# MarbleHE/ABC

Measured on AMD Instinct MI355X. Metric: homomorphic mul+relin/sec, CKKS N=2^14, higher is better.
Workload: dtype u64 (transforms: exact integer arithmetic in f64); 1 GPU; CKKS N=16384, 4 data limbs {50,40,40,40} + special 50-bit prime, ct x ct multiply + relinearize; total_batch=8192, batch_rank0=8192

## Files before the change

abc_amd/csrc/abc_context.hip:

```cpp
#include <cstdlib>
#include <cstring>
#include <mutex>

#include "../../include/abc_hip.h"
#include <dlfcn.h>

#include "abc_context.hpp"
#include "abc_host_math.hpp"
#include "abc_sample.hpp"

namespace abc {

static thread_local std::string g_err;
void set_error(const std::string &msg) { g_err = msg; }

static bool env_on(const char *name) {
  const char *e = std::getenv(name);
  return e && !(e[0] == '0' && e[1] == 0);
}
void read_switches(abc_hip_ctx *c) {
  abc_hip_ctx::Switches s;
  s.no_fused = env_on("ABC_HIP_NO_FUSED");
  s.no_split = env_on("ABC_HIP_NO_SPLIT");
  s.no_split4 = env_on("ABC_HIP_NO_SPLIT4");
  s.no_isplit = env_on("ABC_HIP_NO_ISPLIT");
  s.no_gsplit = env_on("ABC_HIP_NO_GSPLIT");
  s.no_bsplit = env_on("ABC_HIP_NO_BSPLIT");
  s.no_mixed = env_on("ABC_HIP_NO_MIXED");
  s.no_pack = env_on("ABC_HIP_NO_PACK");
  s.no_key_twin = env_on("ABC_HIP_NO_KEY_TWIN");
  s.no_bmul = env_on("ABC_HIP_NO_BMUL");
  s.no_iks = env_on("ABC_HIP_NO_IKS");
  s.no_lean_front = env_on("ABC_HIP_NO_LEAN_FRONT");
  s.no_tensor_intt = env_on("ABC_HIP_NO_TENSOR_INTT");
  s.no_galois_fusion = env_on("ABC_HIP_NO_GALOIS_FUSION");
  s.host_sampling = env_on("ABC_HIP_HOST_SAMPLING");
  if (const char *e = std::getenv("ABC_HIP_CHUNK")) s.chunk = (size_t)std::atol(e);
  if (const char *e = std::getenv("ABC_HIP_FEW_LIMBS")) s.few_limbs = (size_t)std::atol(e);
  if (const char *e = std::getenv("ABC_HIP_LEAN_LIMIT")) s.lean_limit = (size_t)std::atol(e);
  if (const char *e = std::getenv("ABC_HIP_PASS0_TARGET_LIMIT")) s.pass0_target_limit = (size_t)std::atol(e);
  if (const char *e = std::getenv("ABC_HIP_BFV_SCRATCH_MB")) s.bfv_scratch_mb = (size_t)std::atol(e);
  if (const char *e = std::getenv("ABC_HIP_LANES")) {
    s.lanes = std::atoi(e);
    if (s.lanes < 1) s.lanes = 1;
    if (s.lanes > abc_hip_ctx::kMaxLanes) s.lanes = abc_hip_ctx::kMaxLanes;
  }
  c->sw = s;
  RouteFacts &f = c->facts;
  f = RouteFacts{};
  f.scheme = c->scheme; f.logn = c->logn; f.K = c->K; f.L = c->L; f.nB = c->nB;
  f.use_fp = c->use_fp; f.behz_fp = c->behz_fp;
  f.big_block_log = big_block_log();
  for (int j = 0; j < c->K; j++) f.bits[j] = (unsigned char)c->h_mods[j].bits;
  f.sw = s;
  f.finish();
}

static Mod make_mod(uint64_t q, int logn, bool ntt) {
  using namespace host;
  Mod m{};
  m.q = q;
  m.two_q = 2 * q;
  const int k = bitlen(q);
  m.bits = (u32)k;
  m.shift = (u32)(k - 1);
  m.mu = (uint64_t)((((u128)1) << (k + 63)) / q);
  m.qd = (double)q;
  m.qinv = 1.0 / (double)q;
  if (ntt) {
    const uint64_t n = 1ull << logn;
    m.inv_n = invmod(n % q, q);
    m.inv_n_s = shoup(m.inv_n, q);
    if (fp_ok(m.bits)) {
      m.inv_n_c = m.inv_n > q / 2 ? -(double)(q - m.inv_n) : (double)m.inv_n;
      m.inv_n_cq = m.inv_n_c / m.qd;
    }
  }
  return m;
}

static void fill_twiddles(uint64_t q, int logn, uint64_t *dst ) {
  using namespace host;
  const size_t n = (size_t)1 << logn;
  const uint64_t psi = min_primitive_root(2 * n, q);
  uint64_t *fwd = dst, *inv = dst + 2 * n;
  uint64_t p = 1;
  for (size_t i = 0; i < n; i++) {
    fwd[2 * (size_t)bitrev((uint32_t)i, logn)] = p;
    p = mulmod(p, psi, q);
  }
  const uint64_t ipsi = invmod(psi, q);
  p = 1;
  for (size_t i = 0; i < n; i++) {
    inv[2 * (size_t)bitrev((uint32_t)i, logn)] = p;
    p = mulmod(p, ipsi, q);
  }
  for (size_t i = 0; i < n; i++) {
    fwd[2 * i + 1] = shoup(fwd[2 * i], q);
    inv[2 * i + 1] = shoup(inv[2 * i], q);
  }
}

static void fill_fp_twiddles(uint64_t q, size_t n, const uint64_t *src , double *dst ) {
  for (size_t i = 0; i < 2 * n; i++) {
    const uint64_t w = src[2 * i];
    dst[i] = w > q / 2 ? -(double)(q - w) : (double)w;
  }
}

static int build_context(abc_hip_ctx *c) {
  using namespace host;
  const int logn = c->logn, K = c->K, L = c->L;
  const size_t N = (size_t)c->n;
  const bool bfv = (c->scheme == ABC_HIP_SCHEME_BFV);
  std::vector<uint64_t> qs(c->primes.begin(), c->primes.begin() + L);
  const uint64_t qsp = c->primes[K - 1];
  DevConst &k = c->h_cst;
  std::memset(&k, 0, sizeof(k));

  c->mod_values.assign(c->primes.begin(), c->primes.end());
  std::vector<uint64_t> Bp;
  uint64_t m_sk = 0, gamma = 0;
  if (bfv) {
    bool fp_aux = !env_on("ABC_HIP_NO_FP64") && !env_on("ABC_HIP_BEHZ_SEAL_BASE");
    for (uint64_t q : c->primes) fp_aux = fp_aux && fp_ok((u32)bitlen(q));
    const int aux_bits = fp_aux ? 50 : 61;
    int nB = L;
    if (32 + bitlen(c->t) + prod_bitlen(qs) >= aux_bits * L + aux_bits) nB++;
    gamma = ntt_primes(N, 61, 2)[1];
    if (!fp_aux) {
      auto aux = ntt_primes(N, 61, (size_t)nB + 2);
      m_sk = aux[0];
      Bp.assign(aux.begin() + 2, aux.end());
    } else {
      std::vector<uint64_t> alt;
      for (uint64_t p : ntt_primes(N, 50, (size_t)nB + 1 + (size_t)K)) {
        bool clash = false;
        for (uint64_t q : c->primes) clash = clash || (p == q);
        if (!clash && alt.size() < (size_t)nB + 1) alt.push_back(p);
      }
      if (alt.size() < (size_t)nB + 1) throw std::runtime_error("not enough 50-bit NTT primes for the BEHZ auxiliary base");
      m_sk = alt[0];
      Bp.assign(alt.begin() + 1, alt.end());
    }
    c->behz_fp = fp_aux && L <= 10 && !env_on("ABC_HIP_BEHZ_INT_KERNELS");
    c->nB = nB;
    c->nBsk = nB + 1;
    for (uint64_t b : Bp) c->mod_values.push_back(b);
    c->mod_values.push_back(m_sk);
    c->mod_values.push_back(gamma);
    c->mod_values.push_back(c->t);
  }
  const int nmods = (int)c->mod_values.size();
  const int id_bsk = K, id_gamma = K + c->nBsk, id_t = K + c->nBsk + 1;
  c->h_mods.clear();
  std::vector<uint64_t> h_tw((size_t)nmods * 4 * N, 0);
  std::vector<double> h_ftw((size_t)nmods * 2 * N, 0.0);
  for (int i = 0; i < nmods; i++) {
    const bool ntt = !(bfv && i == id_gamma);
    c->h_mods.push_back(make_mod(c->mod_values[i], logn, ntt));
    if (ntt) fill_twiddles(c->mod_values[i], logn, h_tw.data() + (size_t)i * 4 * N);
    if (ntt && fp_ok(c->h_mods.back().bits))
      fill_fp_twiddles(c->mod_values[i], N, h_tw.data() + (size_t)i * 4 * N, h_ftw.data() + (size_t)i * 2 * N);
  }

  for (int j = 0; j < L; j++) {
    const uint64_t q = qs[j];
    k.inv_special[j] = invmod(qsp % q, q);
    k.inv_special_s[j] = shoup(k.inv_special[j], q);
    k.special_mod_q[j] = qsp % q;
    k.special_mod_q_s[j] = shoup(k.special_mod_q[j], q);
    k.inv_special_c[j] = k.inv_special[j] > q / 2 ? -(double)(q - k.inv_special[j]) : (double)k.inv_special[j];
    k.inv_special_cq[j] = k.inv_special_c[j] / (double)q;
    k.special_c[j] = k.special_mod_q[j] > q / 2 ? -(double)(q - k.special_mod_q[j]) : (double)k.special_mod_q[j];
    k.special_cq[j] = k.special_c[j] / (double)q;
  }
  for (int l = 1; l < L; l++)
    for (int j = 0; j < l; j++) {
      k.inv_qlast[l][j] = invmod(qs[l] % qs[j], qs[j]);
      k.inv_qlast_s[l][j] = shoup(k.inv_qlast[l][j], qs[j]);
      k.inv_qlast_c[l][j] = k.inv_qlast[l][j] > qs[j] / 2 ? -(double)(qs[j] - k.inv_qlast[l][j]) : (double)k.inv_qlast[l][j];
      k.inv_qlast_cq[l][j] = k.inv_qlast_c[l][j] / (double)qs[j];
    }

  std::vector<uint32_t> slot_map;
  if (bfv) {
    const uint64_t t = c->t;
    k.t = t;
// ... 767 lines not shown
```

abc_amd/csrc/abc_kernels_fused.hip:

```cpp
#include <type_traits>

#include "abc_context.hpp"
#include "abc_host_math.hpp"

namespace abc {

template <int LB>
__global__ __launch_bounds__((1 << LB) / 16) void k_fused_tensor_intt(DevCtx c, const u64 *__restrict__ a,
                                                                      const u64 *__restrict__ b, u64 *__restrict__ c01,
                                                                      u64 *__restrict__ c2coef, u64 *__restrict__ c2ntt, int nl) {
  __shared__ u64 lds[lds_words(LB)];
  const int j = blockIdx.x % nl;
  const size_t ct = blockIdx.x / nl;
  const size_t N = (size_t)1 << LB, pw = (size_t)nl * N;
  const Mod m = c.mods[j];
  const NttTable t = ntt_table(c, j);
  const u64 *__restrict__ a0 = a + ct * 2 * pw + j * N, *__restrict__ a1 = a0 + pw;
  const u64 *__restrict__ b0 = b + ct * 2 * pw + j * N, *__restrict__ b1 = b0 + pw;
  u64 *__restrict__ o0 = c01 + ct * 2 * pw + j * N, *__restrict__ o1 = o0 + pw;
  u64 *__restrict__ dcoef = c2coef + (ct * nl + j) * N, *__restrict__ dntt = c2ntt + (ct * nl + j) * N;
  ntt_inv_block<LB>(
      lds,
      [&](int, int i) {
        const u64 x0 = a0[i], x1 = a1[i], y0 = b0[i], y1 = b1[i];
// ... 602 lines not shown
  const size_t cc = blockIdx.x >> 2;
  const int p = (int)((blockIdx.x & 3) << 8) + (int)threadIdx.x;
  const int hi0[1] = {0};
  double x[16];
  {
    const Mod ms = mod_at(c, c.K - 1);
    const FpTable ts = fp_table(c, c.K - 1);
    const FpK ks = FpArith::consts(ms);
    const double *__restrict__ src = tsp_half + cc * (size_t)c.ps;
#pragma unroll
    for (int k = 0; k < 16; k++) x[k] = src[(k << 10) + p];
    FpArith::centre16(x, ks);
    inv_pass<FpArith, LB, 0, 4>(x, hi0, ts, ks, 0, 0);
    const double half = (double)(ms.q >> 1);
#pragma unroll
    for (int k = 0; k < 16; k++) {
      const double w = fp_centre(fp_mul_lazy(x[k], ms.inv_n_c, ms.inv_n_cq, ms.qd) + half, ms.qd, ms.qinv);
      x[k] = w < 0.0 ? w + ms.qd : w;
    }
  }
  const u64 half = c.mods[c.K - 1].q >> 1;
  for (int j = 0; j < nl; j++) {
    const Mod m = mod_at(c, j);
    const FpTable t = fp_table(c, j);
    const FpK kk = FpArith::consts(m);
    const u64 hm = reduce64(half, m);
    const double fix = hm ? (double)(m.q - hm) : 0.0;
    double y[16];
#pragma unroll
    for (int k = 0; k < 16; k++) y[k] = x[k] + fix;
    fwd_pass<FpArith, LB, 0, 4>(y, hi0, t, kk, 0, 0);
    double *__restrict__ dst = tpart + (cc * nl + j) * (size_t)c.ps;
    store_half_done<LB>(dst, y, p, kk, pack ? pack_kind(m.bits) : 0);
  }
}

template <int MODE, bool GAL, int NL>
__global__ __launch_bounds__(NL ? (NL + 1) * 64 : 832) void k_split3_main_fp(DevCtx c, const double *__restrict__ part,
                                                                              const double *__restrict__ tpart,
                                                                              const u64 *__restrict__ opa, const u64 *__restrict__ opb,
                                                                              size_t opa_stride, size_t opb_stride, int add_c1,
                                                                              const u64 *__restrict__ key, u64 *__restrict__ out, int nl_rt,
                                                                              u32 gelt) {
  extern __shared__ double dyn[];
  const int nl = NL ? NL : nl_rt;
  const int W = __builtin_amdgcn_readfirstlane((int)(threadIdx.x >> 6));
  const int lane = threadIdx.x & 63;
  const int blk = blockIdx.x & 15;
  const int I = (int)((blockIdx.x >> 4) % nl);
  const size_t ct = (size_t)((blockIdx.x >> 4) / nl);
  const size_t N = (size_t)c.n, base = (size_t)blk << 10;
  const Mod m = mod_at(c, I);
  const FpTable t = fp_table(c, I);
  const double q = m.qd, qinv = m.qinv;
  {
    double *buf = dyn + W * lds_words(10);
    const double *__restrict__ src;
    if (W < nl - 1) {
      const int J = W < I ? W : W + 1;
      src = part + ((ct * (nl + 1) + I) * nl + J) * (size_t)c.ps + base;
    } else {
      src = tpart + ((ct * 2 + (W - (nl - 1))) * nl + I) * (size_t)c.ps + base;
    }
    ntt_fwd_block_a<10, FpArith>(
        buf, [&](int, int i) { return fp_centre(src[i], q, qinv); }, [&](int, int i, double v) { buf[lds_pad(i)] = v; }, t, m, 4, blk,
        lane);
  }
  __syncthreads();
  const double inv = c.cst->inv_special_c[I], inv_q = c.cst->inv_special_cq[I];
  const size_t pw = (size_t)nl * N;
  const double *tt0 = dyn + (nl - 1) * lds_words(10), *tt1 = dyn + nl * lds_words(10);
  for (int e = 2 * (int)threadIdx.x; e < 1024; e += 2 * (int)blockDim.x) {
    double s0[2] = {0.0, 0.0}, s1[2] = {0.0, 0.0}, d0[2] = {0.0, 0.0}, d1[2] = {0.0, 0.0};
#pragma unroll
    for (int Jx = 0; Jx < (NL ? NL : 12); Jx++) {
      if (!NL && Jx >= nl) break;
      double x[2];
      if (Jx == I) {
        if (MODE == 0) {
          const u64 *pa = opa + ct * 2 * pw + (size_t)I * N + base + e, *pb = opb + ct * 2 * pw + (size_t)I * N + base + e;
          const u64x2 a0 = *reinterpret_cast<const u64x2 *>(pa), a1 = *reinterpret_cast<const u64x2 *>(pa + pw);
          const u64x2 b0 = *reinterpret_cast<const u64x2 *>(pb), b1 = *reinterpret_cast<const u64x2 *>(pb + pw);
          const double x0[2] = {fp_from_u64(a0.x), fp_from_u64(a0.y)}, x1[2] = {fp_from_u64(a1.x), fp_from_u64(a1.y)};
          const double y0[2] = {fp_from_u64(b0.x), fp_from_u64(b0.y)}, y1[2] = {fp_from_u64(b1.x), fp_from_u64(b1.y)};
#pragma unroll
          for (int k = 0; k < 2; k++) {
            x[k] = fp_mulmod(x1[k], y1[k], q, qinv);
            d0[k] = fp_mulmod(x0[k], y0[k], q, qinv);
            d1[k] = fp_mulmod(x0[k], y1[k], q, qinv) + fp_mulmod(x1[k], y0[k], q, qinv);
          }
        } else {
          const u64 *xl = opa + ct * opa_stride + (size_t)I * N;
#pragma unroll
          for (int k = 0; k < 2; k++) {
            const u32 si = galois_ntt_src<GAL>((u32)(base + e + k), gelt, c.logn);
            x[k] = fp_from_u64(xl[si]);
            if (opb) {
              const u64 *ad = opb + ct * opb_stride + (size_t)I * N;
              d0[k] = fp_from_u64(ad[si]);
              if (add_c1) d1[k] = fp_from_u64(ad[pw + si]);
            }
          }
        }
      } else {
        const int w = Jx < I ? Jx : Jx - 1;
        const f64x2 v = *reinterpret_cast<const f64x2 *>(dyn + w * lds_words(10) + lds_pad(e));
        x[0] = v.x;
        x[1] = v.y;
      }
      const u64x2 k0 = *reinterpret_cast<const u64x2 *>(key + (((size_t)Jx * 2 + 0) * c.K + I) * N + base + e);
      const u64x2 k1 = *reinterpret_cast<const u64x2 *>(key + (((size_t)Jx * 2 + 1) * c.K + I) * N + base + e);
      s0[0] += fp_mulmod(x[0], fp_from_u64(k0.x), q, qinv);
      s0[1] += fp_mulmod(x[1], fp_from_u64(k0.y), q, qinv);
      s1[0] += fp_mulmod(x[0], fp_from_u64(k1.x), q, qinv);
      s1[1] += fp_mulmod(x[1], fp_from_u64(k1.y), q, qinv);
      if (Jx == 7) {
#pragma unroll
        for (int k = 0; k < 2; k++) {
          s0[k] = fp_centre(s0[k], q, qinv);
          s1[k] = fp_centre(s1[k], q, qinv);
        }
      }
    }
    const f64x2 u0 = *reinterpret_cast<const f64x2 *>(tt0 + lds_pad(e)), u1 = *reinterpret_cast<const f64x2 *>(tt1 + lds_pad(e));
    u64x2 r;
    r.x = fp_to_canon(fp_mul_lazy(s0[0] - u0.x, inv, inv_q, q) + d0[0], q, qinv);
    r.y = fp_to_canon(fp_mul_lazy(s0[1] - u0.y, inv, inv_q, q) + d0[1], q, qinv);
    *reinterpret_cast<u64x2 *>(out + ((ct * 2 + 0) * nl + I) * N + base + e) = r;
    r.x = fp_to_canon(fp_mul_lazy(s1[0] - u1.x, inv, inv_q, q) + d1[0], q, qinv);
    r.y = fp_to_canon(fp_mul_lazy(s1[1] - u1.y, inv, inv_q, q) + d1[1], q, qinv);
    *reinterpret_cast<u64x2 *>(out + ((ct * 2 + 1) * nl + I) * N + base + e) = r;
  }
}

template <int MODE, bool GAL>
static void launch_split3_main(abc_hip_ctx *c, const MainArgs &a) {
  const int nl = a.nl;
  const dim3 grid((unsigned)(a.cc * nl * 16)), block(64 * (nl + 1));
  const size_t lds = (size_t)((nl + 1) * lds_words(10)) * 8;
#define ABC_TM3(NLV)                                                                                                             \
  hipLaunchKernelGGL((k_split3_main_fp<MODE, GAL, NLV>), grid, block, lds, a.st, c->dc, (const double *)a.part, (const double *)a.tpart, \
                     a.opa, a.opb, a.opa_stride, a.opb_stride, a.add_c1, a.key, a.out, nl, a.gelt)
  switch (nl) {
    case 1: ABC_TM3(1); break;
    case 2: ABC_TM3(2); break;
    case 3: ABC_TM3(3); break;
    case 4: ABC_TM3(4); break;
    default: ABC_TM3(0); break;
  }
#undef ABC_TM3
}


template <int MODE, int NL>
struct PairOps {
  u64x2 k0[NL], k1[NL];
  u64x2 a0, a1, b0, b1;
  u64 xs[2], d0s[2], d1s[2];
};

template <int MODE, bool GAL, int NL>
__global__ __launch_bounds__(512, NL <= 4 ? 4 : 2) void k_split4_main_fp(DevCtx c, const double *__restrict__ part,
                                                                   const double *__restrict__ tpart, const u64 *__restrict__ opa,
                                                                   const u64 *__restrict__ opb, size_t opa_stride, size_t opb_stride,
                                                                   int add_c1, const u64 *__restrict__ key, u64 *__restrict__ out, u32 gelt,
                                                                   u32 imap, int ni, int pack, const double *__restrict__ keyf) {
  extern __shared__ double dyn[];
  static_assert(NL + 1 <= 8, "one wavefront per limb, eight wavefronts");
  constexpr int nl = NL, NT = 512, PER = 2;
  constexpr int LATE = (MODE == 0 && NL == 4) ? 1 : 0;
  const int W = __builtin_amdgcn_readfirstlane((int)(threadIdx.x >> 6));
  const int lane = threadIdx.x & 63;
  const int blk = blockIdx.x & 15;
  const int I = (int)((imap >> (4 * ((blockIdx.x >> 4) % (unsigned)ni))) & 15u);
  const size_t ct = (size_t)((blockIdx.x >> 4) / (unsigned)ni);
  const size_t N = (size_t)c.n, base = (size_t)blk << 10;
  const Mod m = mod_at(c, I);
  const FpTable t = fp_table(c, I);
  const double q = m.qd, qinv = m.qinv;
  double *ltw = dyn + (nl + 1) * lds_words(10);
  const size_t pw = (size_t)nl * N;
  const ABC_CONST_AS DevConst *cst = (const ABC_CONST_AS DevConst *)c.cst;
  const double inv = cst->inv_special_c[I], inv_q = cst->inv_special_cq[I];

  double twv[PER];
  block_twiddles_fetch<10, double, PER>(t.tw, 4, blk, (int)threadIdx.x, NT, twv);
  const bool has_limb = W <= nl;
  const int Wc = has_limb ? W : 0;
  const double *__restrict__ src = (Wc < nl - 1) ? part + ((ct * (nl + 1) + I) * nl + (Wc < I ? Wc : Wc + 1)) * (size_t)c.ps + base
                                                 : tpart + ((ct * 2 + (Wc - (nl - 1))) * nl + I) * (size_t)c.ps + base;
  const int pk = pack ? pack_kind(m.bits) : 0;
  u64x2 raw[8];
  if (has_limb) {
    if (pk == 0) {
#pragma unroll
      for (int k = 0; k < 8; k++) raw[k] = *reinterpret_cast<const u64x2 *>(src + (k << 7) + 2 * lane);
    } else if (pk == 1) {
#pragma unroll
      for (int k = 0; k < 8; k++) raw[k] = pack_load_pair<1>(src - base, N, base + (k << 7) + 2 * lane);
    } else {
#pragma unroll
      for (int k = 0; k < 8; k++) raw[k] = pack_load_pair<2>(src - base, N, base + (k << 7) + 2 * lane);
    }
  }
  auto load_key = [&](int e, PairOps<MODE, NL> &o, int j0, int j1) {
    const u64 *kw = keyf ? reinterpret_cast<const u64 *>(keyf) : key;
#pragma unroll
    for (int Jx = 0; Jx < NL; Jx++) {
      if (Jx < j0 || Jx >= j1) continue;
      o.k0[Jx] = *reinterpret_cast<const u64x2 *>(kw + (((size_t)Jx * 2 + 0) * c.K + I) * N + base + e);
      o.k1[Jx] = *reinterpret_cast<const u64x2 *>(kw + (((size_t)Jx * 2 + 1) * c.K + I) * N + base + e);
    }
  };
  auto load_pair = [&](int e, PairOps<MODE, NL> &o) {
    load_key(e, o, 0, NL - LATE);
    if (MODE == 0) {
      const u64 *pa = opa + ct * 2 * pw + (size_t)I * N + base + e, *pb = opb + ct * 2 * pw + (size_t)I * N + base + e;
      o.a0 = *reinterpret_cast<const u64x2 *>(pa); o.a1 = *reinterpret_cast<const u64x2 *>(pa + pw);
      o.b0 = *reinterpret_cast<const u64x2 *>(pb); o.b1 = *reinterpret_cast<const u64x2 *>(pb + pw);
    } else {
      const u64 *xl = opa + ct * opa_stride + (size_t)I * N;
#pragma unroll
      for (int k = 0; k < 2; k++) {
        const u32 si = galois_ntt_src<GAL>((u32)(base + e + k), gelt, c.logn);
        o.xs[k] = xl[si];
        o.d0s[k] = o.d1s[k] = 0;
        if (opb) {
          const u64 *ad = opb + ct * opb_stride + (size_t)I * N;
          o.d0s[k] = ad[si];
          if (add_c1) o.d1s[k] = ad[pw + si];
        }
      }
    }
  };
  PairOps<MODE, NL> ops;
  load_pair(2 * (int)threadIdx.x, ops);

  block_twiddles_store<10, double, PER>(ltw, (int)threadIdx.x, NT, twv);
  __syncthreads();
  if (has_limb) {
    double *buf = dyn + W * lds_words(10);
    double xin[16];
    if (pk == 0) {
#pragma unroll
      for (int k = 0; k < 8; k++) {
        xin[k] = __longlong_as_double((long long)raw[k].x);
        xin[8 + k] = __longlong_as_double((long long)raw[k].y);
      }
    } else if (pk == 1) {
#pragma unroll
      for (int k = 0; k < 8; k++) pack_decode_pair<1>(raw[k], xin[k], xin[8 + k]);
    } else {
#pragma unroll
      for (int k = 0; k < 8; k++) pack_decode_pair<2>(raw[k], xin[k], xin[8 + k]);
    }
    if (m.bits >= 49) {
#pragma unroll
      for (int r = 0; r < 16; r++) xin[r] = fp_centre(xin[r], q, qinv);
    }
    ntt_fwd_tail1024_pairs<FpTail>(buf, xin, [&](int, int i, double v) { buf[lds_pad(i)] = v; }, t, m, 4, blk, lane, ltw);
  }
  if (LATE) load_key(2 * (int)threadIdx.x, ops, NL - LATE, NL);
  __syncthreads();
  const double *tt0 = dyn + (nl - 1) * lds_words(10), *tt1 = dyn + nl * lds_words(10);
  auto compute_pair = [&](int e, const PairOps<MODE, NL> &o, auto twin) {
    constexpr bool TW = decltype(twin)::value;
    auto kd = [](u64 w) { return TW ? __longlong_as_double((long long)w) : fp_from_u64(w); };
    double s0[2] = {0.0, 0.0}, s1[2] = {0.0, 0.0}, d0[2] = {0.0, 0.0}, d1[2] = {0.0, 0.0};
#pragma unroll
    for (int Jx = 0; Jx < NL; Jx++) {
      double x[2];
      if (Jx == I) {
        if (MODE == 0) {
          const double x0[2] = {fp_from_u64(o.a0.x), fp_from_u64(o.a0.y)}, x1[2] = {fp_from_u64(o.a1.x), fp_from_u64(o.a1.y)};
          const double y0[2] = {fp_from_u64(o.b0.x), fp_from_u64(o.b0.y)}, y1[2] = {fp_from_u64(o.b1.x), fp_from_u64(o.b1.y)};
#pragma unroll
          for (int k = 0; k < 2; k++) {
            x[k] = fp_mulmod(x1[k], y1[k], q, qinv);
            d0[k] = fp_mulmod(x0[k], y0[k], q, qinv);
            d1[k] = fp_mulmod(x0[k], y1[k], q, qinv) + fp_mulmod(x1[k], y0[k], q, qinv);
          }
        } else {
#pragma unroll
          for (int k = 0; k < 2; k++) {
            x[k] = fp_from_u64(o.xs[k]);
            d0[k] = fp_from_u64(o.d0s[k]);
            d1[k] = fp_from_u64(o.d1s[k]);
          }
        }
      } else {
        const int w = Jx < I ? Jx : Jx - 1;
        const f64x2 v = *reinterpret_cast<const f64x2 *>(dyn + w * lds_words(10) + lds_pad(e));
        x[0] = v.x;
        x[1] = v.y;
      }
      s0[0] += fp_mulmod(x[0], kd(o.k0[Jx].x), q, qinv);
      s0[1] += fp_mulmod(x[1], kd(o.k0[Jx].y), q, qinv);
      s1[0] += fp_mulmod(x[0], kd(o.k1[Jx].x), q, qinv);
      s1[1] += fp_mulmod(x[1], kd(o.k1[Jx].y), q, qinv);
      if (Jx == 7) {
#pragma unroll
        for (int k = 0; k < 2; k++) {
          s0[k] = fp_centre(s0[k], q, qinv);
          s1[k] = fp_centre(s1[k], q, qinv);
        }
      }
    }
    const f64x2 u0 = *reinterpret_cast<const f64x2 *>(tt0 + lds_pad(e)), u1 = *reinterpret_cast<const f64x2 *>(tt1 + lds_pad(e));
    u64x2 r;
    r.x = fp_to_canon(fp_mul_lazy(s0[0] - u0.x, inv, inv_q, q) + d0[0], q, qinv);
    r.y = fp_to_canon(fp_mul_lazy(s0[1] - u0.y, inv, inv_q, q) + d0[1], q, qinv);
    *reinterpret_cast<u64x2 *>(out + ((ct * 2 + 0) * nl + I) * N + base + e) = r;
    r.x = fp_to_canon(fp_mul_lazy(s1[0] - u1.x, inv, inv_q, q) + d1[0], q, qinv);
    r.y = fp_to_canon(fp_mul_lazy(s1[1] - u1.y, inv, inv_q, q) + d1[1], q, qinv);
    *reinterpret_cast<u64x2 *>(out + ((ct * 2 + 1) * nl + I) * N + base + e) = r;
  };
  if (keyf) compute_pair(2 * (int)threadIdx.x, ops, std::true_type{});
  else compute_pair(2 * (int)threadIdx.x, ops, std::false_type{});
}

bool split4_main(abc_hip_ctx *c, int mode, const MainArgs &a) {
  if (a.nl < 1 || a.nl > 7) return false;
  if (a.ni == 0) return true;
  const dim3 grid((unsigned)(a.cc * a.ni * 16)), block(512);
  const double *keyf = key_twin_lookup(c, a.key);
  dispatch_mode(mode, a.gelt, [&](auto M, auto G) {
    dispatch_nl<1, 7>(a.nl, [&](auto NL) {
      hipLaunchKernelGGL((k_split4_main_fp<decltype(M)::value, decltype(G)::value, decltype(NL)::value>), grid, block, main_lds_bytes(a.nl, sizeof(double)),
                         a.st, c->dc, (const double *)a.part, (const double *)a.tpart, a.opa, a.opb, a.opa_stride, a.opb_stride, a.add_c1,
                         a.key, a.out, a.gelt, (u32)a.imap, a.ni, a.pack, keyf);
    });
  });
  return true;
}

static void launch_split3(abc_hip_ctx *c, const FusedScratch &s, int mode, MainArgs a, bool main4) {
  a.part = s.dec;
  a.tpart = s.ksacc;
  launch_split_special(a.st, c, a.cc, a.nl, (const double *)s.dec, a.key, (double *)s.tsp);
  hipLaunchKernelGGL(k_split3_pass_fp<14>, dim3((unsigned)(a.cc * 2 * 4)), dim3(256), 0, a.st, c->dc, (const double *)s.tsp,
                     (double *)s.ksacc, a.nl, a.pack);
  if (main4 && split4_main(c, mode, a)) return;
  dispatch_mode(mode, a.gelt, [&](auto M, auto G) { launch_split3_main<decltype(M)::value, decltype(G)::value>(c, a); });
}

template <int LB>
static int keyswitch_stage(abc_hip_ctx *c, hipStream_t st, const FusedScratch &s, const u64 *coef, size_t coef_stride, const u64 *ntt,
                           size_t ntt_stride, const u64 *key, const u64 *addend, size_t addend_stride, bool add_c1, u64 *out, int nl,
                           size_t cc, bool fp , const ChunkRoute &k,
                           int dec_ready = 0 ) {
  const size_t N = (size_t)1 << LB;
  const dim3 block((1 << LB) / 16);
  const bool ckks = (c->scheme == 2);
  const bool guard = k.guard, lazy = k.lazy;
  const unsigned g2a = (unsigned)(cc * (nl + 1) * nl);
  const unsigned g3 = (unsigned)(cc * 2 * nl);
  if (fp) {
    if (!dec_ready)
      hipLaunchKernelGGL(k_fused_ks_decomp_ntt_fp<LB>, dim3(g2a), block, 0, st, c->dc, coef, coef_stride, s.dec, nl, ckks ? 1 : 0);
    hipLaunchKernelGGL(k_fused_ks_mac, dim3(grid_for(cc * (nl + 1) * (N / 2), 256)), dim3(256), 0, st, c->dc, s.dec,
                       ckks ? ntt : (const u64 *)nullptr, ntt_stride, key, s.ksacc, s.tsp, nl, cc);
    hipLaunchKernelGGL(k_fused_ks_special_intt_fp<LB>, dim3((unsigned)(cc * 2)), block, 0, st, c->dc, s.tsp, s.tlast);
    if (ckks)
      hipLaunchKernelGGL((k_fused_ks_moddown_fp<LB, false>), dim3(g3), block, 0, st, c->dc, s.ksacc, s.tlast, addend, addend_stride,
                         add_c1 ? 1 : 0, out, nl, (int)(cc * 2), 0u);
    else
      hipLaunchKernelGGL(k_fused_ks_moddown_bfv_fp<LB>, dim3(g3), block, 0, st, c->dc, s.ksacc, s.tlast, addend, addend_stride,
                         add_c1 ? 1 : 0, out, nl);
    ABC_HIP_CHECK(hipGetLastError());
    return 0;
  }
  if (guard)
    hipLaunchKernelGGL((k_fused_ks_decomp_ntt<LB, true, false>), dim3(g2a), block, 0, st, c->dc, coef, coef_stride, s.dec, nl,
                       ckks ? 1 : 0);
  else if (lazy)
    hipLaunchKernelGGL((k_fused_ks_decomp_ntt<LB, false, true>), dim3(g2a), block, 0, st, c->dc, coef, coef_stride, s.dec, nl,
                       ckks ? 1 : 0);
  else
    hipLaunchKernelGGL((k_fused_ks_decomp_ntt<LB, false, false>), dim3(g2a), block, 0, st, c->dc, coef, coef_stride, s.dec, nl,
                       ckks ? 1 : 0);
  hipLaunchKernelGGL(k_fused_ks_mac, dim3(grid_for(cc * (nl + 1) * (N / 2), 256)), dim3(256), 0, st, c->dc, s.dec,
                     ckks ? ntt : (const u64 *)nullptr, ntt_stride, key, s.ksacc, s.tsp, nl, cc);
  hipLaunchKernelGGL(k_fused_ks_special_intt<LB>, dim3((unsigned)(cc * 2)), block, 0, st, c->dc, s.tsp, s.tlast);
  if (!ckks)
    hipLaunchKernelGGL(k_fused_ks_moddown_bfv<LB>, dim3(g3), block, 0, st, c->dc, s.ksacc, s.tlast, addend, addend_stride,
                       add_c1 ? 1 : 0, out, nl);
  else if (guard)
    hipLaunchKernelGGL((k_fused_ks_moddown<LB, true>), dim3(g3), block, 0, st, c->dc, s.ksacc, s.tlast, addend, addend_stride,
                       add_c1 ? 1 : 0, out, nl);
  else
    hipLaunchKernelGGL((k_fused_ks_moddown<LB, false>), dim3(g3), block, 0, st, c->dc, s.ksacc, s.tlast, addend, addend_stride,
                       add_c1 ? 1 : 0, out, nl);
  ABC_HIP_CHECK(hipGetLastError());
  return 0;
}

int fork_lanes(abc_hip_ctx *c, int lanes) {
  if (lanes < 2) return 0;
  ABC_HIP_CHECK(hipEventRecord(c->lane_fork, c->stream));
  for (int l = 0; l < lanes; l++) ABC_HIP_CHECK(hipStreamWaitEvent(c->lane[l], c->lane_fork, 0));
  return 0;
}
int join_lanes(abc_hip_ctx *c, int lanes) {
  if (lanes < 2) return 0;
  for (int l = 0; l < lanes; l++) {
    ABC_HIP_CHECK(hipEventRecord(c->lane_join[l], c->lane[l]));
    ABC_HIP_CHECK(hipStreamWaitEvent(c->stream, c->lane_join[l], 0));
  }
  return 0;
}

static int run_isplit(abc_hip_ctx *c, int mode, const u64 *opa, const u64 *opb, size_t opa_stride, size_t opb_stride, bool add_c1,
                      const u64 *key, u64 *out, int nl, size_t count, u32 gelt) {
  const size_t N = (size_t)c->n;
  const ChunkPlan p = plan_chunks(c->facts, nl, count);
  const ChunkRoute k = route_chunk(c->facts, Seq::isplit, nl, p.chunk);
  return for_each_chunk(c, count, p.chunk, p.lanes, isplit_scratch_words(c, nl), k.fp_twin ? key : nullptr,
                        [&](hipStream_t st, u64 *scratch, size_t off, size_t cc) {
                          return isplit_chunk(c, st, scratch, cc, nl, mode, opa + off * opa_stride, opb ? opb + off * opb_stride : nullptr,
                                              opa_stride, opb_stride, add_c1 ? 1 : 0, key, out + off * 2 * (size_t)nl * N, gelt, k);
                        });
}

static int run_gsplit15(abc_hip_ctx *c, int mode, const u64 *opa, const u64 *opb, size_t opa_stride, size_t opb_stride, bool add_c1,
                        const u64 *key, u64 *out, int nl, size_t count, u32 gelt) {
  const size_t N = (size_t)c->n;
  const ChunkPlan p = plan_chunks(c->facts, nl, count);
  return for_each_chunk(c, count, p.chunk, p.lanes, gsplit_scratch_words(c, nl), nullptr,
                        [&](hipStream_t st, u64 *scratch, size_t off, size_t cc) {
                          return gsplit_chunk15(c, st, scratch, cc, nl, mode, opa + off * opa_stride, opb ? opb + off * opb_stride : nullptr,
                                                opa_stride, opb_stride, add_c1 ? 1 : 0, key, out + off * 2 * (size_t)nl * N, gelt);
                        });
}

template <int LB>
static int run_mul_relin(abc_hip_ctx *c, Seq seq, const u64 *a, const u64 *b, u64 *out, int nl, size_t count) {
  const size_t N = (size_t)1 << LB;
  const ChunkPlan p = plan_chunks(c->facts, nl, count);
  const bool split = seq == Seq::split14, fp = seq != Seq::lds_int;
  const size_t SN = split ? (size_t)c->dc.ps : N;
  const size_t per_ct = fused_scratch_limbs(nl) * SN;
  const size_t ctw = 2 * (size_t)nl * N;
  return for_each_chunk(c, count, p.chunk, p.lanes, per_ct, split ? c->d_relin : nullptr, [&](hipStream_t st, u64 *scratch, size_t off, size_t cc) {
    const FusedScratch s = carve(scratch, p.chunk, nl, SN);
    const ChunkRoute k = route_chunk(c->facts, seq, nl, cc);
    if constexpr (LB == 14) {
      if (split) {
        if (k.lean)
          gsplit_front14(st, c, cc, nl, 0, a + off * ctw, b + off * ctw, 0, (double *)s.coef, (double *)s.dec, 0u, k.pack);
        else
          hipLaunchKernelGGL(k_split2_tensor_pass0_fp<LB>, dim3((unsigned)(cc * nl)), dim3((1 << LB) / 16), 0, st, c->dc, a + off * ctw,
                             b + off * ctw, (double *)s.dec, nl, (int)k.pack);
        launch_split3(c, s, 0, MainArgs{st, cc, nl, nullptr, nullptr, a + off * ctw, b + off * ctw, 0, 0, 0, c->d_relin, out + off * ctw, 0u,
                                        kAllSlots, nl, k.pack},
                      k.main4);
        ABC_HIP_CHECK(hipGetLastError());
        return 0;
      }
    }
    if (fp)
      hipLaunchKernelGGL(k_fused_tensor_decomp_fp<LB>, dim3((unsigned)(cc * nl)), dim3((1 << LB) / 16), 0, st, c->dc, a + off * ctw,
                         b + off * ctw, s.c01, s.ntt, s.dec, nl);
    else
      hipLaunchKernelGGL(k_fused_tensor_intt<LB>, dim3((unsigned)(cc * nl)), dim3((1 << LB) / 16), 0, st, c->dc, a + off * ctw,
                         b + off * ctw, s.c01, s.coef, s.ntt, nl);
    return keyswitch_stage<LB>(c, st, s, s.coef, (size_t)nl * N, s.ntt, (size_t)nl * N, c->d_relin, s.c01, ctw, true, out + off * ctw, nl,
                               cc, fp, k, fp ? 1 : 0);
  });
}

int launch_mul_relin(abc_hip_ctx *c, Seq seq, const u64 *a, const u64 *b, u64 *out, int nl, size_t count) {
  if (!count) return 0;
  const size_t ctw = 2 * (size_t)nl * c->n;
  switch (seq) {
    case Seq::gsplit15: return run_gsplit15(c, 0, a, b, ctw, ctw, false, c->d_relin, out, nl, count, 0u);
    case Seq::isplit: return run_isplit(c, 0, a, b, ctw, ctw, false, c->d_relin, out, nl, count, 0u);
    case Seq::split14:
    case Seq::lds_fp:
    case Seq::lds_int: return dispatch_logn<10, 14>(c->logn, [&](auto LB) { return run_mul_relin<decltype(LB)::value>(c, seq, a, b, out, nl, count); });
    default: set_error("launch_mul_relin: not a multiply + relinearise sequence of this file"); return 1;
  }
}

// ... 79 lines not shown
```

abc_amd/csrc/abc_route.hpp:

```cpp
#pragma once

#include <cstddef>
#include <cstdint>
#include <cstdio>

namespace abc {

struct Switches {
  bool no_fused = false, no_split = false, no_split4 = false, no_isplit = false, no_gsplit = false, no_lean_front = false, no_bsplit = false, no_mixed = false, no_pack = false, no_key_twin = false, no_bmul = false, no_iks = false, no_tensor_intt = false;
  bool no_galois_fusion = false;
  bool host_sampling = false;
  size_t chunk = 0, few_limbs = 48, lean_limit = 96, bfv_scratch_mb = 0, pass0_target_limit = 128;
  int lanes = 2;
};

constexpr unsigned kFpBits = 50;
constexpr unsigned kLazyBits = 55;
constexpr unsigned kUnguardedBits = 57;
constexpr unsigned kIsplitBits = 60;

constexpr size_t fused_scratch_limbs(int nl) { return (size_t)nl * (nl + 1) + 6 * (size_t)nl + 4; }

struct RouteFacts {
  int scheme = 0, logn = 0, K = 0, L = 0, nB = 0;
  bool use_fp = true, behz_fp = false;
  int big_block_log = 12;
  unsigned char bits[17] = {};
  Switches sw;
  unsigned widest = 0;
  uint32_t fp_mask = 0;
  bool all_fp = false;
  bool guard = false;
  bool lazy = false;
  void finish() {
    widest = 0;
    fp_mask = 0;
    for (int j = 0; j < K; j++) {
      if (bits[j] > widest) widest = bits[j];
      if (bits[j] <= kFpBits) fp_mask |= 1u << j;
    }
    all_fp = use_fp && widest <= kFpBits;
    guard = widest > kUnguardedBits;
    lazy = widest <= kLazyBits;
  }
  uint32_t fp_data_mask(int nl) const { return fp_mask & ((1u << nl) - 1u); }
  bool data_fp(int nl) const { return fp_data_mask(nl) == (1u << nl) - 1u; }
  bool special_fp() const { return K > 0 && ((fp_mask >> (K - 1)) & 1u); }
};

enum class Seq {
  split14,
  gsplit15,
  isplit,
  bsplit14,
  bsplit_big,
  lds_fp,
  lds_int,
  bmul,
  generic
};
enum class KsFront { plain, fp, iks };
enum class BfvMul { behz, split, big };
enum class Rescale { generic, fp, mixed };

struct KsRoute {
  Seq seq;
  KsFront front;
};
struct MulRoute {
  Seq seq;
  BfvMul mul;
  KsRoute ks;
};
struct RotRoute {
  bool fold;
  KsRoute ks;
};
struct RescaleRoute {
  Rescale kind;
  uint32_t fpmask;
};

namespace route_detail {
inline bool gsplit_ok(const RouteFacts &f, int nl) {
  return f.logn == 15 && f.scheme == 2 && f.use_fp && !f.sw.no_gsplit && nl >= 1 && nl <= 15 && f.widest <= kFpBits;
}
inline bool bsplit_ok(const RouteFacts &f, int nl) {
  return f.logn == 14 && f.scheme == 1 && f.use_fp && !f.sw.no_bsplit && nl >= 1 && nl <= 8 && f.widest <= kFpBits;
}
inline bool bsplit_big_ok(const RouteFacts &f, int nl) {
  return (f.logn == 13 || f.logn == 15 || f.logn == 16) && f.scheme == 1 && f.use_fp && !f.sw.no_bsplit && !f.sw.no_gsplit && nl >= 1 &&
         nl <= 8 && f.widest <= kFpBits;
}
inline bool isplit_ok(const RouteFacts &f, int nl) {
  if ((f.logn != 14 && f.logn != 15) || f.scheme != 2 || f.sw.no_fused || f.sw.no_split || f.sw.no_isplit || nl < 1 ||
      nl > (f.logn == 15 ? 15 : 7))
    return false;
  if (f.logn == 15 && f.sw.no_gsplit) return false;
  return f.widest <= kIsplitBits;
}
inline bool bmul_shape(const RouteFacts &f, int limbs) {
  return f.scheme == 1 && f.use_fp && f.behz_fp && !f.sw.no_bmul && !f.sw.no_split && !f.sw.no_fused && f.L == limbs && f.nB == limbs &&
         f.K == f.L + 1;
}
inline bool bmul_relin_ok(const RouteFacts &f) {
  if (f.logn == 13) return bmul_shape(f, 4) && bsplit_big_ok(f, f.L);
  return f.logn == 14 && bmul_shape(f, 8) && bsplit_ok(f, f.L);
}
inline Seq lds_seq(const RouteFacts &f, int nl, bool mul) {
  const bool ckks = f.scheme == 2;
  if (f.logn == 14 && ckks && !f.all_fp && isplit_ok(f, nl)) return Seq::isplit;
  if (f.logn == 14 && ckks && f.all_fp && !f.sw.no_split && nl <= 12) return Seq::split14;
  if (!mul && f.logn == 14 && !ckks && !f.sw.no_split && bsplit_ok(f, nl)) return Seq::bsplit14;
  return f.all_fp ? Seq::lds_fp : Seq::lds_int;
}
}

inline KsFront route_ks_front(const RouteFacts &f, int nl) {
  if (f.logn > 14 && f.use_fp && f.data_fp(nl) && f.special_fp()) return KsFront::fp;
  if ((f.logn == 15 || f.logn == 16) && !f.sw.no_iks && f.big_block_log == 12) return KsFront::iks;
  return KsFront::plain;
}

inline KsRoute route_keyswitch(const RouteFacts &f, int nl) {
  using namespace route_detail;
  const KsRoute generic{Seq::generic, route_ks_front(f, nl)};
  if (f.logn == 15 && gsplit_ok(f, nl)) return {Seq::gsplit15, KsFront::plain};
  if (f.logn == 15 && f.scheme == 2 && !f.all_fp && isplit_ok(f, nl)) return {Seq::isplit, KsFront::plain};
  if (bsplit_big_ok(f, nl)) return {Seq::bsplit_big, KsFront::plain};
  if (f.logn > 14 || f.logn < 10 || f.sw.no_fused) return generic;
  return {lds_seq(f, nl, false), KsFront::plain};
}

inline BfvMul route_bfv_multiply(const RouteFacts &f) {
  using namespace route_detail;
  if (f.logn == 14) return bmul_relin_ok(f) ? BfvMul::split : BfvMul::behz;
  if (f.logn == 13) return bmul_shape(f, 4) ? BfvMul::big : BfvMul::behz;
  return ((f.logn == 15 || f.logn == 16) && bmul_shape(f, 8) && !f.sw.no_gsplit && f.big_block_log == 12) ? BfvMul::big : BfvMul::behz;
}

inline MulRoute route_mul_relin(const RouteFacts &f, int nl) {
  using namespace route_detail;
  const KsRoute none{Seq::generic, KsFront::plain};
  if (f.scheme == 2) {
    if (f.logn == 15 && gsplit_ok(f, nl)) return {Seq::gsplit15, BfvMul::behz, none};
    if (f.logn == 15 && !f.all_fp && isplit_ok(f, nl)) return {Seq::isplit, BfvMul::behz, none};
    if (f.logn <= 14 && f.logn >= 10 && !f.sw.no_fused) return {lds_seq(f, nl, true), BfvMul::behz, none};
    return {Seq::generic, BfvMul::behz, route_keyswitch(f, nl)};
  }
  if (bmul_relin_ok(f)) return {Seq::bmul, BfvMul::split, none};
  return {Seq::generic, route_bfv_multiply(f), route_keyswitch(f, nl)};
}

inline RotRoute route_rotate(const RouteFacts &f, int nl, bool in_place) {
  using namespace route_detail;
  const bool may_fold = !in_place && !f.sw.no_galois_fusion;
  if (may_fold && f.logn == 15 && gsplit_ok(f, nl)) return {true, {Seq::gsplit15, KsFront::plain}};
  if (may_fold && f.logn == 15 && f.scheme == 2 && !f.all_fp && isplit_ok(f, nl)) return {true, {Seq::isplit, KsFront::plain}};
  if (may_fold && f.scheme == 1) {
    if (!f.sw.no_split && !f.sw.no_fused) {
      if (f.logn == 14 && bsplit_ok(f, nl)) return {true, {Seq::bsplit14, KsFront::plain}};
      if (bsplit_big_ok(f, nl)) return {true, {Seq::bsplit_big, KsFront::plain}};
    }
// ... 114 lines not shown
```

Measured before the change: 419,000 mul+relin/s.

## Split key-switch main kernel into two output halves for three workgroups per CU

For four or fewer limbs, the split4 main kernel now holds only one key component at a time in registers. It computes the first output component, then reloads the second key component and computes the second. Key and operand loads are also deferred until after the forward NTT, and launch bounds are raised so more workgroups fit per CU. In exchange it adds a second pass over the LDS digits, puts key loads on the critical path, and lets the old schedule be restored with an environment switch.

Measured after the change: 436,000 mul+relin/s, median of 6. 4.1% higher.

```diff
diff --git a/abc_amd/csrc/abc_context.hip b/abc_amd/csrc/abc_context.hip
--- a/abc_amd/csrc/abc_context.hip
+++ b/abc_amd/csrc/abc_context.hip
@@ -34,6 +34,7 @@
   s.no_lean_front = env_on("ABC_HIP_NO_LEAN_FRONT");
   s.no_tensor_intt = env_on("ABC_HIP_NO_TENSOR_INTT");
   s.no_galois_fusion = env_on("ABC_HIP_NO_GALOIS_FUSION");
+  s.main_two_per_cu = env_on("ABC_HIP_MAIN_TWO_PER_CU");
   s.host_sampling = env_on("ABC_HIP_HOST_SAMPLING");
   if (const char *e = std::getenv("ABC_HIP_CHUNK")) s.chunk = (size_t)std::atol(e);
   if (const char *e = std::getenv("ABC_HIP_FEW_LIMBS")) s.few_limbs = (size_t)std::atol(e);
diff --git a/abc_amd/csrc/abc_kernels_fused.hip b/abc_amd/csrc/abc_kernels_fused.hip
--- a/abc_amd/csrc/abc_kernels_fused.hip
+++ b/abc_amd/csrc/abc_kernels_fused.hip
@@ -778,23 +778,25 @@
 }
 
 
-template <int MODE, int NL>
+template <int MODE, int NL, bool HALVES>
 struct PairOps {
-  u64x2 k0[NL], k1[NL];
+  u64x2 k[HALVES ? NL : 2 * NL];
   u64x2 a0, a1, b0, b1;
   u64 xs[2], d0s[2], d1s[2];
 };
 
-template <int MODE, bool GAL, int NL>
-__global__ __launch_bounds__(512, NL <= 4 ? 4 : 2) void k_split4_main_fp(DevCtx c, const double *__restrict__ part,
+template <int MODE, bool GAL, int NL, bool HALVES>
+__global__ __launch_bounds__(512, HALVES ? 6 : NL <= 4 ? 4 : 2) void k_split4_main_fp(DevCtx c, const double *__restrict__ part,
                                                                    const double *__restrict__ tpart, const u64 *__restrict__ opa,
                                                                    const u64 *__restrict__ opb, size_t opa_stride, size_t opb_stride,
                                                                    int add_c1, const u64 *__restrict__ key, u64 *__restrict__ out, u32 gelt,
                                                                    u32 imap, int ni, int pack, const double *__restrict__ keyf) {
   extern __shared__ double dyn[];
   static_assert(NL + 1 <= 8, "one wavefront per limb, eight wavefronts");
+  static_assert(!HALVES || NL <= 4, "three workgroups per CU: four transform buffers at the most");
   constexpr int nl = NL, NT = 512, PER = 2;
-  constexpr int LATE = (MODE == 0 && NL == 4) ? 1 : 0;
+  constexpr int LATE = (!HALVES && MODE == 0 && NL == 4) ? 1 : 0;
+  using Ops = PairOps<MODE, NL, HALVES>;
   const int W = __builtin_amdgcn_readfirstlane((int)(threadIdx.x >> 6));
   const int lane = threadIdx.x & 63;
   const int blk = blockIdx.x & 15;
@@ -829,17 +831,20 @@
       for (int k = 0; k < 8; k++) raw[k] = pack_load_pair<2>(src - base, N, base + (k << 7) + 2 * lane);
     }
   }
-  auto load_key = [&](int e, PairOps<MODE, NL> &o, int j0, int j1) {
+  auto load_key = [&](int e, Ops &o, int j0, int j1, int comp) {
     const u64 *kw = keyf ? reinterpret_cast<const u64 *>(keyf) : key;
 #pragma unroll
     for (int Jx = 0; Jx < NL; Jx++) {
       if (Jx < j0 || Jx >= j1) continue;
-      o.k0[Jx] = *reinterpret_cast<const u64x2 *>(kw + (((size_t)Jx * 2 + 0) * c.K + I) * N + base + e);
-      o.k1[Jx] = *reinterpret_cast<const u64x2 *>(kw + (((size_t)Jx * 2 + 1) * c.K + I) * N + base + e);
+      if constexpr (HALVES) {
+        o.k[Jx] = *reinterpret_cast<const u64x2 *>(kw + (((size_t)Jx * 2 + comp) * c.K + I) * N + base + e);
+      } else {
+        o.k[2 * Jx + 0] = *reinterpret_cast<const u64x2 *>(kw + (((size_t)Jx * 2 + 0) * c.K + I) * N + base + e);
+        o.k[2 * Jx + 1] = *reinterpret_cast<const u64x2 *>(kw + (((size_t)Jx * 2 + 1) * c.K + I) * N + base + e);
+      }
     }
   };
-  auto load_pair = [&](int e, PairOps<MODE, NL> &o) {
-    load_key(e, o, 0, NL - LATE);
+  auto load_operands = [&](int e, Ops &o) {
     if (MODE == 0) {
       const u64 *pa = opa + ct * 2 * pw + (size_t)I * N + base + e, *pb = opb + ct * 2 * pw + (size_t)I * N + base + e;
       o.a0 = *reinterpret_cast<const u64x2 *>(pa); o.a1 = *reinterpret_cast<const u64x2 *>(pa + pw);
@@ -859,8 +864,12 @@
       }
     }
   };
-  PairOps<MODE, NL> ops;
-  load_pair(2 * (int)threadIdx.x, ops);
+  Ops ops;
+  const int e0 = 2 * (int)threadIdx.x;
+  if (!HALVES) {
+    load_key(e0, ops, 0, NL - LATE, 0);
+    load_operands(e0, ops);
+  }
 
   block_twiddles_store<10, double, PER>(ltw, (int)threadIdx.x, NT, twv);
   __syncthreads();
@@ -886,63 +895,97 @@
     }
     ntt_fwd_tail1024_pairs<FpTail>(buf, xin, [&](int, int i, double v) { buf[lds_pad(i)] = v; }, t, m, 4, blk, lane, ltw);
   }
-  if (LATE) load_key(2 * (int)threadIdx.x, ops, NL - LATE, NL);
+  if (HALVES) {
+    load_key(e0, ops, 0, NL, 0);
+    load_operands(e0, ops);
+  }
+  if (LATE) load_key(e0, ops, NL - LATE, NL, 0);
   __syncthreads();
-  const double *tt0 = dyn + (nl - 1) * lds_words(10), *tt1 = dyn + nl * lds_words(10);
-  auto compute_pair = [&](int e, const PairOps<MODE, NL> &o, auto twin) {
+  auto compute_pair = [&](int e, Ops &o, auto twin) {
     constexpr bool TW = decltype(twin)::value;
     auto kd = [](u64 w) { return TW ? __longlong_as_double((long long)w) : fp_from_u64(w); };
-    double s0[2] = {0.0, 0.0}, s1[2] = {0.0, 0.0}, d0[2] = {0.0, 0.0}, d1[2] = {0.0, 0.0};
-#pragma unroll
-    for (int Jx = 0; Jx < NL; Jx++) {
-      double x[2];
-      if (Jx == I) {
-        if (MODE == 0) {
-          const double x0[2] = {fp_from_u64(o.a0.x), fp_from_u64(o.a0.y)}, x1[2] = {fp_from_u64(o.a1.x), fp_from_u64(o.a1.y)};
-          const double y0[2] = {fp_from_u64(o.b0.x), fp_from_u64(o.b0.y)}, y1[2] = {fp_from_u64(o.b1.x), fp_from_u64(o.b1.y)};
+    double xd[2], d0[2] = {0.0, 0.0}, d1[2] = {0.0, 0.0};
+    auto diagonal = [&]() {
+      if (MODE == 0) {
+        const double x0[2] = {fp_from_u64(o.a0.x), fp_from_u64(o.a0.y)}, x1[2] = {fp_from_u64(o.a1.x), fp_from_u64(o.a1.y)};
+        const double y0[2] = {fp_from_u64(o.b0.x), fp_from_u64(o.b0.y)}, y1[2] = {fp_from_u64(o.b1.x), fp_from_u64(o.b1.y)};
+#pragma unroll
+        for (int k = 0; k < 2; k++) {
+          xd[k] = fp_mulmod(x1[k], y1[k], q, qinv);
+          d0[k] = fp_mulmod(x0[k], y0[k], q, qinv);
+          d1[k] = fp_mulmod(x0[k], y1[k], q, qinv) + fp_mulmod(x1[k], y0[k], q, qinv);
+        }
+      } else {
+#pragma unroll
+        for (int k = 0; k < 2; k++) {
+          xd[k] = fp_from_u64(o.xs[k]);
+          d0[k] = fp_from_u64(o.d0s[k]);
+          d1[k] = fp_from_u64(o.d1s[k]);
+        }
+      }
+    };
+    auto digit = [&](int Jx, double *x) {
+      const int w = Jx < I ? Jx : Jx - 1;
+      const f64x2 v = *reinterpret_cast<const f64x2 *>(dyn + w * lds_words(10) + lds_pad(e));
+      x[0] = v.x;
+      x[1] = v.y;
+    };
+    auto finish = [&](int comp, const double *s, const double *d) {
+      const f64x2 u = *reinterpret_cast<const f64x2 *>(dyn + (nl - 1 + comp) * lds_words(10) + lds_pad(e));
+      u64x2 r;
+      r.x = fp_to_canon(fp_mul_lazy(s[0] - u.x, inv, inv_q, q) + d[0], q, qinv);
+      r.y = fp_to_canon(fp_mul_lazy(s[1] - u.y, inv, inv_q, q) + d[1], q, qinv);
+      *reinterpret_cast<u64x2 *>(out + ((ct * 2 + comp) * nl + I) * N + base + e) = r;
+    };
+    if constexpr (HALVES) {
+      diagonal();
+#pragma unroll
+      for (int k = 0; k < 2; k++) asm volatile("" : "+v"(xd[k]), "+v"(d0[k]), "+v"(d1[k]));
+      auto half = [&](auto comp, const double *d) {
+        double s[2] = {0.0, 0.0};
+#pragma unroll
+        for (int Jx = 0; Jx < NL; Jx++) {
+          double x[2] = {xd[0], xd[1]};
+          if (Jx != I) digit(Jx, x);
+          s[0] += fp_mulmod(x[0], kd(o.k[Jx].x), q, qinv);
+          s[1] += fp_mulmod(x[1], kd(o.k[Jx].y), q, qinv);
+        }
+        finish(decltype(comp)::value, s, d);
+      };
+      half(std::integral_constant<int, 0>{}, d0);
+      __builtin_amdgcn_sched_barrier(0);
+      load_key(e, o, 0, NL, 1);
+      half(std::integral_constant<int, 1>{}, d1);
+    } else {
+      double s0[2] = {0.0, 0.0}, s1[2] = {0.0, 0.0};
+#pragma unroll
+      for (int Jx = 0; Jx < NL; Jx++) {
+        double x[2];
+        if (Jx == I) {
+          diagonal();
+          x[0] = xd[0];
+          x[1] = xd[1];
+        } else {
+          digit(Jx, x);
+        }
+        s0[0] += fp_mulmod(x[0], kd(o.k[2 * Jx + 0].x), q, qinv);
+        s0[1] += fp_mulmod(x[1], kd(o.k[2 * Jx + 0].y), q, qinv);
+        s1[0] += fp_mulmod(x[0], kd(o.k[2 * Jx + 1].x), q, qinv);
+        s1[1] += fp_mulmod(x[1], kd(o.k[2 * Jx + 1].y), q, qinv);
+        if (Jx == 7) {
 #pragma unroll
           for (int k = 0; k < 2; k++) {
-            x[k] = fp_mulmod(x1[k], y1[k], q, qinv);
-            d0[k] = fp_mulmod(x0[k], y0[k], q, qinv);
-            d1[k] = fp_mulmod(x0[k], y1[k], q, qinv) + fp_mulmod(x1[k], y0[k], q, qinv);
-          }
-        } else {
-#pragma unroll
-          for (int k = 0; k < 2; k++) {
-            x[k] = fp_from_u64(o.xs[k]);
-            d0[k] = fp_from_u64(o.d0s[k]);
-            d1[k] = fp_from_u64(o.d1s[k]);
+            s0[k] = fp_centre(s0[k], q, qinv);
+            s1[k] = fp_centre(s1[k], q, qinv);
           }
         }
-      } else {
-        const int w = Jx < I ? Jx : Jx - 1;
-        const f64x2 v = *reinterpret_cast<const f64x2 *>(dyn + w * lds_words(10) + lds_pad(e));
-        x[0] = v.x;
-        x[1] = v.y;
-      }
-      s0[0] += fp_mulmod(x[0], kd(o.k0[Jx].x), q, qinv);
-      s0[1] += fp_mulmod(x[1], kd(o.k0[Jx].y), q, qinv);
-      s1[0] += fp_mulmod(x[0], kd(o.k1[Jx].x), q, qinv);
-      s1[1] += fp_mulmod(x[1], kd(o.k1[Jx].y), q, qinv);
-      if (Jx == 7) {
-#pragma unroll
-        for (int k = 0; k < 2; k++) {
-          s0[k] = fp_centre(s0[k], q, qinv);
-          s1[k] = fp_centre(s1[k], q, qinv);
-        }
-      }
-    }
-    const f64x2 u0 = *reinterpret_cast<const f64x2 *>(tt0 + lds_pad(e)), u1 = *reinterpret_cast<const f64x2 *>(tt1 + lds_pad(e));
-    u64x2 r;
-    r.x = fp_to_canon(fp_mul_lazy(s0[0] - u0.x, inv, inv_q, q) + d0[0], q, qinv);
-    r.y = fp_to_canon(fp_mul_lazy(s0[1] - u0.y, inv, inv_q, q) + d0[1], q, qinv);
-    *reinterpret_cast<u64x2 *>(out + ((ct * 2 + 0) * nl + I) * N + base + e) = r;
-    r.x = fp_to_canon(fp_mul_lazy(s1[0] - u1.x, inv, inv_q, q) + d1[0], q, qinv);
-    r.y = fp_to_canon(fp_mul_lazy(s1[1] - u1.y, inv, inv_q, q) + d1[1], q, qinv);
-    *reinterpret_cast<u64x2 *>(out + ((ct * 2 + 1) * nl + I) * N + base + e) = r;
+      }
+      finish(0, s0, d0);
+      finish(1, s1, d1);
+    }
   };
-  if (keyf) compute_pair(2 * (int)threadIdx.x, ops, std::true_type{});
-  else compute_pair(2 * (int)threadIdx.x, ops, std::false_type{});
+  if (keyf) compute_pair(e0, ops, std::true_type{});
+  else compute_pair(e0, ops, std::false_type{});
 }
 
 bool split4_main(abc_hip_ctx *c, int mode, const MainArgs &a) {
@@ -952,9 +995,15 @@
   const double *keyf = key_twin_lookup(c, a.key);
   dispatch_mode(mode, a.gelt, [&](auto M, auto G) {
     dispatch_nl<1, 7>(a.nl, [&](auto NL) {
-      hipLaunchKernelGGL((k_split4_main_fp<decltype(M)::value, decltype(G)::value, decltype(NL)::value>), grid, block, main_lds_bytes(a.nl, sizeof(double)),
-                         a.st, c->dc, (const double *)a.part, (const double *)a.tpart, a.opa, a.opb, a.opa_stride, a.opb_stride, a.add_c1,
-                         a.key, a.out, a.gelt, (u32)a.imap, a.ni, a.pack, keyf);
+      auto launch = [&](auto H) {
+        hipLaunchKernelGGL((k_split4_main_fp<decltype(M)::value, decltype(G)::value, decltype(NL)::value, decltype(H)::value>), grid, block,
+                           main_lds_bytes(a.nl, sizeof(double)), a.st, c->dc, (const double *)a.part, (const double *)a.tpart, a.opa, a.opb,
+                           a.opa_stride, a.opb_stride, a.add_c1, a.key, a.out, a.gelt, (u32)a.imap, a.ni, a.pack, keyf);
+      };
+      if constexpr (decltype(NL)::value <= 4) {
+        if (!c->sw.main_two_per_cu) return launch(std::true_type{});
+      }
+      launch(std::false_type{});
     });
   });
   return true;
diff --git a/abc_amd/csrc/abc_route.hpp b/abc_amd/csrc/abc_route.hpp
--- a/abc_amd/csrc/abc_route.hpp
+++ b/abc_amd/csrc/abc_route.hpp
@@ -9,6 +9,7 @@
 struct Switches {
   bool no_fused = false, no_split = false, no_split4 = false, no_isplit = false, no_gsplit = false, no_lean_front = false, no_bsplit = false, no_mixed = false, no_pack = false, no_key_twin = false, no_bmul = false, no_iks = false, no_tensor_intt = false;
   bool no_galois_fusion = false;
+  bool main_two_per_cu = false;
   bool host_sampling = false;
   size_t chunk = 0, few_limbs = 48, lean_limit = 96, bfv_scratch_mb = 0, pass0_target_limit = 128;
   int lanes = 2;
```
